# JuliaMolSim/DFTK.jl

Measured on NVIDIA H100. Metric: hpsi_band_applies_per_s, higher is better.
Workload: dtype f64

## Files before the change

### dftk.jl_b200/csrc/fft.cu

```cuda
#include "structs.cuh"

namespace dftk {

#define FFT_THREADS 256
extern __shared__ __align__(16) unsigned char dyn_smem[];

__global__ void __launch_bounds__(FFT_THREADS)
k_sphere_to_x(SphereTables T, FftPlan px, const cplx* twx, const cplx* psi, int64_t ldpsi, cplx* W1,
              int L, int Lp) {
  stage_sphere_to_x(T, px, twx, psi, ldpsi, W1, L, Lp, (cplx*)dyn_smem,
                    Dim3i{(int)blockIdx.x, (int)blockIdx.y, 0});
}
__global__ void __launch_bounds__(FFT_THREADS)
k_y_backward(SphereTables T, FftPlan py, const cplx* twy, const cplx* W1, cplx* W2, int L, int Lp) {
  stage_y_backward(T, py, twy, W1, W2, L, Lp, (cplx*)dyn_smem,
                   Dim3i{(int)blockIdx.x, (int)blockIdx.y, (int)blockIdx.z});
}
__global__ void __launch_bounds__(FFT_THREADS)
k_z_apply_potential(SphereTables T, FftPlan pz, const cplx* twz, cplx* W2, const double* V, int L,
                    int Lp) {
  stage_z_apply_potential(T, pz, twz, W2, V, L, Lp, (cplx*)dyn_smem,
                          Dim3i{(int)blockIdx.x, (int)blockIdx.y, (int)blockIdx.z});
}
__global__ void __launch_bounds__(FFT_THREADS)
// ... 153 lines not shown
  dftk_b200_ctx* ctx = g->ctx;
  ensure_scratch(kb, nb);
  if ((g->rx && kb->T.ranges_ok)) {
    int L = reg_L(g->rx), Lp = L + 1;
    const cplx* tw = (const cplx*)g->twx.p;
    cplx* W1 = kb->W1.p;
    void* args[] = {&kb->T, &tw, &psi, &ldpsi, &W1, &L, &Lp};
    launch_ptr(ctx, g->rx->sphere_to_x, dim3(cdiv(kb->T.n_cols, L), nb), L * g->rx->T, reg_smem(g->rx) + 5 * L * sizeof(int), args);
  } else {
    int L = g->Lx, Lp = L | 1;
    LAUNCH(ctx, k_sphere_to_x, dim3(cdiv(kb->T.n_cols, L), nb), FFT_THREADS, smem_for(g->nx, L), kb->T,
           g->px, (const cplx*)g->twx.p, psi, ldpsi, kb->W1.p, L, Lp);
  }
  if ((g->ry && kb->T.ranges_ok)) {
    int L = reg_L(g->ry), Lp = L + 1;
    const cplx* tw = (const cplx*)g->twy.p;
    const cplx* W1 = kb->W1.p;
    cplx* W2 = kb->W2.p;
    void* args[] = {&kb->T, &tw, &W1, &W2, &L, &Lp};
    launch_ptr(ctx, g->ry->y_backward, dim3(cdiv(g->nx, L), kb->T.n_zc, nb), L * g->ry->T, reg_smem(g->ry), args);
  } else {
    int L = g->Ly, Lp = L | 1;
    LAUNCH(ctx, k_y_backward, dim3(cdiv(g->nx, L), kb->T.n_zc, nb), FFT_THREADS, smem_for(g->ny, L),
           kb->T, g->py, (const cplx*)g->twy.p, (const cplx*)kb->W1.p, kb->W2.p, L, Lp);
  }
}

void kb_planes_to_sphere(dftk_b200_kblock* kb, cplx* out, int64_t ldout, int nb, double scale,
                         const double* kin, const cplx* psi, int64_t ldpsi, int accumulate) {
  dftk_b200_grid* g = kb->grid;
  dftk_b200_ctx* ctx = g->ctx;
  if ((g->ry && kb->T.ranges_ok)) {
    int L = reg_L(g->ry), Lp = L + 1;
    const cplx* tw = (const cplx*)g->twy.p;
    const cplx* W2 = kb->W2.p;
    cplx* W1 = kb->W1.p;
    void* args[] = {&kb->T, &tw, &W2, &W1, &L, &Lp};
    launch_ptr(ctx, g->ry->y_forward, dim3(cdiv(g->nx, L), kb->T.n_zc, nb), L * g->ry->T, reg_smem(g->ry), args);
  } else {
    int L = g->Ly, Lp = L | 1;
    LAUNCH(ctx, k_y_forward, dim3(cdiv(g->nx, L), kb->T.n_zc, nb), FFT_THREADS, smem_for(g->ny, L),
           kb->T, g->py, (const cplx*)g->twy.p, (const cplx*)kb->W2.p, kb->W1.p, L, Lp);
  }
  if ((g->rx && kb->T.ranges_ok)) {
    int L = reg_L(g->rx), Lp = L + 1;
    const cplx* tw = (const cplx*)g->twx.p;
    const cplx* W1 = kb->W1.p;
    void* args[] = {&kb->T, &tw, &W1, &out, &ldout, &scale, &kin, &psi, &ldpsi, &accumulate, &L, &Lp};
    launch_ptr(ctx, g->rx->x_to_sphere, dim3(cdiv(kb->T.n_cols, L), nb), L * g->rx->T, reg_smem(g->rx) + 5 * L * sizeof(int), args);
  } else {
    int L = g->Lx, Lp = L | 1;
    LAUNCH(ctx, k_x_to_sphere, dim3(cdiv(kb->T.n_cols, L), nb), FFT_THREADS, smem_for(g->nx, L), kb->T,
           g->px, (const cplx*)g->twx.p, (const cplx*)kb->W1.p, out, ldout, scale, kin, psi, ldpsi,
           accumulate, L, Lp);
  }
}

void kb_apply_local_kinetic(dftk_b200_kblock* kb, const cplx* psi, cplx* hpsi, int64_t n_bands,
                            bool with_local, bool with_kin, bool accumulate) {
  dftk_b200_grid* g = kb->grid;
  dftk_b200_ctx* ctx = g->ctx;
  if (n_bands == 0) return;
  if (!with_local) {
    scale_kin_add(ctx, psi, hpsi, with_kin ? kb->kin.p : nullptr, kb->n_pw, n_bands, accumulate);
    return;
  }
  REQUIRE(kb->has_V, "apply_h: local potential not set (dftk_b200_kblock_set_potential)");
  const bool fused = kb_yz_fused(kb);
  const int chunk = band_chunk_for(kb, n_bands, !fused);
  for (int64_t b0 = 0; b0 < n_bands; b0 += chunk) {
    int nb = (int)std::min<int64_t>(chunk, n_bands - b0);
    const cplx* p = psi + b0 * kb->n_pw;
    if (fused) {
      kb->W1.ensure((size_t)nb * kb->Th.n_cols * g->nx);
      int L = reg_L(g->rx), Lp = L + 1;
      const size_t sm_x = reg_smem(g->rx) + 5 * L * sizeof(int);
      const cplx* twx = (const cplx*)g->twx.p;
      const cplx* twy = (const cplx*)g->twy.p;
      cplx* W1 = kb->W1.p;
      int64_t ld = kb->n_pw;
      void* a1[] = {&kb->T, &twx, &p, &ld, &W1, &L, &Lp};
      launch_ptr(ctx, g->rx->sphere_to_xt, dim3(cdiv(kb->T.n_cols, L), nb), L * g->rx->T, sm_x, a1);
      const double* Vt = kb->Vtp();
      void* a2[] = {&kb->T, &twy, &W1, &Vt};
      launch_ptr(ctx, g->ry->yz_apply, dim3(nb, g->nx), kYzLines * g->ry->T, yz_smem(g->ny, kb->T.n_zc), a2);
      cplx* out = hpsi + b0 * kb->n_pw;
      double scale = 1.0;
      const double* kin = with_kin ? kb->kin.p : nullptr;
      int acc = accumulate ? 1 : 0;
      void* a3[] = {&kb->T, &twx, &W1, &out, &ld, &scale, &kin, &p, &ld, &acc, &L, &Lp};
      launch_ptr(ctx, g->rx->xt_to_sphere, dim3(cdiv(kb->T.n_cols, L), nb), L * g->rx->T, sm_x, a3);
      continue;
    }
    kb_sphere_to_planes(kb, p, kb->n_pw, nb);
    if ((g->rz && kb->T.ranges_ok)) {
      int L = reg_L(g->rz), Lp = L + 1;
      const cplx* tw = (const cplx*)g->twz.p;
      cplx* W2 = kb->W2.p;
      const double* V = kb->Vp();
      void* args[] = {&kb->T, &tw, &W2, &V, &L, &Lp};
      const size_t sm_pipe = reg_smem(g->rz) / 2 + 2 * (size_t)kb->T.n_zc * L * sizeof(cplx);
      const int64_t n_tiles = (int64_t)cdiv(g->nx, L) * g->ny * nb;
      if (ctx->z_pipeline && sm_pipe <= 100 * 1024 && n_tiles >= 2 * (int64_t)ctx->sm_count) {
        int per_sm = (int)std::min<size_t>(4, (size_t)(220 * 1024) / sm_pipe);
        unsigned grid = (unsigned)std::min<int64_t>(n_tiles, (int64_t)per_sm * ctx->sm_count);
        void* pargs[] = {&kb->T, &tw, &W2, &V, &nb};
        launch_ptr(ctx, g->rz->z_apply_pipe, dim3(grid), L * g->rz->T, sm_pipe, pargs);
      } else {
        launch_ptr(ctx, g->rz->z_apply, dim3(cdiv(g->nx, L), g->ny, nb), L * g->rz->T, reg_smem(g->rz) / 2, args);
      }
    } else {
      int L = g->Lz, Lp = L | 1;
      LAUNCH(ctx, k_z_apply_potential, dim3(cdiv(g->nx, L), g->ny, nb), FFT_THREADS, smem_for(g->nz, L),
             kb->T, g->pz, (const cplx*)g->twz.p, kb->W2.p, (const double*)kb->Vp(), L, Lp);
    }
    kb_planes_to_sphere(kb, hpsi + b0 * kb->n_pw, kb->n_pw, nb, 1.0, with_kin ? kb->kin.p : nullptr, p,
                        kb->n_pw, accumulate ? 1 : 0);
  }
}

bool kb_apply_local_kinetic_multi(int n, dftk_b200_kblock* const* kbs, const cplx* const* psi, cplx* const* hpsi,
                                  const int* n_bands, const void* (*upload)(void* self, const void* host, size_t bytes), void* self) {
  if (n <= 0) return true;
  dftk_b200_grid* g = kbs[0]->grid;
  dftk_b200_ctx* ctx = g->ctx;
  if (!(g->rx && g->ry && g->rz)) return false;
  int total = 0, max_cols = 0, max_zc = 0;
  for (int i = 0; i < n; ++i) {
    dftk_b200_kblock* kb = kbs[i];
    if (kb->grid != g || !kb->T.ranges_ok || !kb->has_V || !kb->has_kin || n_bands[i] <= 0) return false;
    if (band_chunk_for(kb, n_bands[i]) < n_bands[i]) return false;
    total += n_bands[i];
    max_cols = std::max(max_cols, kb->T.n_cols);
    max_zc = std::max(max_zc, kb->T.n_zc);
  }
  if (total > 65535) return false;
  std::vector<FftMultiItem> items(n);
  std::vector<int2> bandmap(total);
  int b = 0;
  for (int i = 0; i < n; ++i) {
    dftk_b200_kblock* kb = kbs[i];
    ensure_scratch(kb, n_bands[i]);
    FftMultiItem& it = items[i];
    it.T = kb->T;
    it.psi = psi[i];
    it.ldpsi = kb->n_pw;
    it.W1 = kb->W1.p;
    it.W2 = kb->W2.p;
    it.V = kb->Vp();
    it.wts = nullptr;
    it.nb = n_bands[i];
    it.out = hpsi[i];
    it.ldout = kb->n_pw;
    it.kin = kb->kin.p;
    for (int l = 0; l < n_bands[i]; ++l) bandmap[b++] = make_int2(i, l);
  }
  const FftMultiItem* d_items = (const FftMultiItem*)upload(self, items.data(), items.size() * sizeof(FftMultiItem));
  const int2* d_map = (const int2*)upload(self, bandmap.data(), bandmap.size() * sizeof(int2));
  {
    int L = reg_L(g->rx), Lp = L + 1;
    const cplx* tw = (const cplx*)g->twx.p;
    void* args[] = {&d_items, &d_map, &tw, &L, &Lp};
    launch_ptr(ctx, g->rx->m_sphere_to_x, dim3(cdiv(max_cols, L), total), L * g->rx->T, reg_smem(g->rx) + 5 * L * sizeof(int), args);
  }
  {
    int L = reg_L(g->ry), Lp = L + 1;
    const cplx* tw = (const cplx*)g->twy.p;
    void* args[] = {&d_items, &d_map, &tw, &L, &Lp};
// ... 184 lines not shown
```

### dftk.jl_b200/csrc/fft_core.cuh

```cuda
#pragma once
#include <cuda_runtime.h>
#include <stdint.h>

#if defined(__CUDA_ARCH__)
#define TLOOP(t, n) for (int t = threadIdx.x; t < (n); t += blockDim.x)
#define TSYNC() __syncthreads()
#else
#define TLOOP(t, n) for (int t = 0; t < (n); ++t)
#define TSYNC() ((void)0)
#endif
#if defined(__CUDA_ARCH__)
#define TLOOPC(t, n, nthr)                                                        \
  _Pragma("unroll") for (int i__ = 0; i__ < ((n) + (nthr)-1) / (nthr); ++i__)    \
      for (int t = (int)threadIdx.x + i__ * (nthr), once__ = 1; once__ && t < (n); once__ = 0)
#define TLOOPU(t, n) _Pragma("unroll 4") for (int t = threadIdx.x; t < (n); t += blockDim.x)
#else
#define TLOOPC(t, n, nthr) for (int t = 0; t < (n); ++t)
#define TLOOPU(t, n) for (int t = 0; t < (n); ++t)
#endif
#define HD __host__ __device__ __forceinline__

namespace dftk {

typedef double2 cplx;

HD cplx cmul(cplx a, cplx b) { return make_double2(a.x * b.x - a.y * b.y, a.x * b.y + a.y * b.x); }
HD cplx cadd(cplx a, cplx b) { return make_double2(a.x + b.x, a.y + b.y); }
HD cplx csub(cplx a, cplx b) { return make_double2(a.x - b.x, a.y - b.y); }
HD cplx cscale(cplx a, double s) { return make_double2(a.x * s, a.y * s); }
HD cplx cmuli(cplx a, double s) { return make_double2(-s * a.y, s * a.x); }

#define DFTK_MAX_PASSES 12
struct FftPlan {
  int n;
  int npass;
  int radix[DFTK_MAX_PASSES];
};

HD cplx twiddle(const cplx* __restrict__ tw, int m, int sign) {
  cplx w = tw[m];
  if (sign > 0) w.y = -w.y;
  return w;
}

template <int R>
HD void butterfly(cplx* v, int sign) {
  const double s = (double)sign;
  if (R == 2) {
    cplx a = v[0], b = v[1];
    v[0] = cadd(a, b);
    v[1] = csub(a, b);
  } else if (R == 4) {
    cplx t0 = cadd(v[0], v[2]), t1 = csub(v[0], v[2]);
    cplx t2 = cadd(v[1], v[3]), t3 = cmuli(csub(v[1], v[3]), s);
    v[0] = cadd(t0, t2);
    v[2] = csub(t0, t2);
    v[1] = cadd(t1, t3);
    v[3] = csub(t1, t3);
  } else if (R == 3) {
    const double h = 0.86602540378443864676;
    cplx t1 = cadd(v[1], v[2]);
    cplx m = make_double2(v[0].x - 0.5 * t1.x, v[0].y - 0.5 * t1.y);
    cplx d = cmuli(cscale(csub(v[1], v[2]), h), s);
    v[0] = cadd(v[0], t1);
    v[1] = cadd(m, d);
    v[2] = csub(m, d);
  } else if (R == 5) {
    const double c1 = 0.30901699437494742410, c2 = -0.80901699437494742410;
    const double s1 = 0.95105651629515357212, s2 = 0.58778525229247312917;
    cplx t1 = cadd(v[1], v[4]), t2 = cadd(v[2], v[3]);
    cplx t3 = csub(v[1], v[4]), t4 = csub(v[2], v[3]);
    cplx m1 = make_double2(v[0].x + c1 * t1.x + c2 * t2.x, v[0].y + c1 * t1.y + c2 * t2.y);
    cplx m2 = make_double2(v[0].x + c2 * t1.x + c1 * t2.x, v[0].y + c2 * t1.y + c1 * t2.y);
    cplx n1 = cmuli(make_double2(s1 * t3.x + s2 * t4.x, s1 * t3.y + s2 * t4.y), s);
    cplx n2 = cmuli(make_double2(s2 * t3.x - s1 * t4.x, s2 * t3.y - s1 * t4.y), s);
    v[0] = cadd(v[0], cadd(t1, t2));
    v[1] = cadd(m1, n1);
    v[4] = csub(m1, n1);
    v[2] = cadd(m2, n2);
    v[3] = csub(m2, n2);
  }
}

template <int R>
HD void stockham_pass(const cplx* __restrict__ in, cplx* __restrict__ out, int n, int Ns, int L,
                      int Lp, const cplx* __restrict__ tw, int sign) {
  const int nb = n / R;
  const int tstep = n / (Ns * R);
  TLOOP(t, nb * L) {
    int line = t % L, j = t / L;
    int k = j % Ns;
    cplx v[R];
#pragma unroll
    for (int r = 0; r < R; ++r) {
      cplx x = in[(j + r * nb) * Lp + line];
      v[r] = (r == 0 || k == 0) ? x : cmul(x, twiddle(tw, r * k * tstep, sign));
    }
    butterfly<R>(v, sign);
    int j0 = (j / Ns) * Ns * R + k;
#pragma unroll
    for (int r = 0; r < R; ++r) out[(j0 + r * Ns) * Lp + line] = v[r];
// ... 325 lines not shown
```

### dftk.jl_b200/csrc/fft_reg.cu

```cuda
#include "structs.cuh"
#include "fft_reg.cuh"

#ifndef REG_GROUP
#define REG_GROUP 0
#endif
#ifndef REG_NGROUPS
#define REG_NGROUPS 1
#endif

namespace dftk {

extern __shared__ __align__(16) unsigned char dyn_smem_reg[];
#define REG_MAXT(A, B) (32 * ((A) > (B) ? (A) : (B)))

template <int A, int B, int XM>
__global__ void __launch_bounds__(REG_MAXT(A, B))
kr_sphere_to_x(SphereTablesX T, const cplx* tw, const cplx* psi, int64_t ldpsi, cplx* W1, int L, int Lp) {
  reg_sphere_to_x<A, B, XM>(T, tw, psi, ldpsi, W1, L, Lp, (cplx*)dyn_smem_reg, Dim3i{(int)blockIdx.x, (int)blockIdx.y, 0});
}
template <int A, int B>
__global__ void __launch_bounds__(REG_MAXT(A, B))
kr_y_backward(SphereTablesX T, const cplx* tw, const cplx* W1, cplx* W2, int L, int Lp) {
  reg_y_backward<A, B>(T, tw, W1, W2, L, Lp, (cplx*)dyn_smem_reg, Dim3i{(int)blockIdx.x, (int)blockIdx.y, (int)blockIdx.z});
}
template <int A, int B>
__global__ void __launch_bounds__(REG_MAXT(A, B))
kr_z_apply(SphereTablesX T, const cplx* tw, cplx* W2, const double* V, int L, int Lp) {
  reg_z_apply_potential<A, B>(T, tw, W2, V, L, Lp, (cplx*)dyn_smem_reg, Dim3i{(int)blockIdx.x, (int)blockIdx.y, (int)blockIdx.z});
}
template <int A, int B>
__global__ void __launch_bounds__(REG_MAXT(A, B))
kr_z_apply_pipe(SphereTablesX T, const cplx* tw, cplx* W2, const double* V, int n_bands) {
  reg_z_apply_potential_pipe<A, B>(T, tw, W2, V, (cplx*)dyn_smem_reg, n_bands);
}
template <int A, int B>
__global__ void __launch_bounds__(REG_MAXT(A, B))
kr_z_to_cube(SphereTablesX T, const cplx* tw, const cplx* W2, cplx* cube, double scale, int L, int Lp) {
  reg_z_to_cube<A, B>(T, tw, W2, cube, scale, L, Lp, (cplx*)dyn_smem_reg, Dim3i{(int)blockIdx.x, (int)blockIdx.y, (int)blockIdx.z});
}
template <int A, int B>
__global__ void __launch_bounds__(REG_MAXT(A, B))
kr_z_from_cube(SphereTablesX T, const cplx* tw, const cplx* cube, cplx* W2, int L, int Lp) {
  reg_z_from_cube<A, B>(T, tw, cube, W2, L, Lp, (cplx*)dyn_smem_reg, Dim3i{(int)blockIdx.x, (int)blockIdx.y, (int)blockIdx.z});
}
template <int A, int B>
__global__ void __launch_bounds__(REG_MAXT(A, B))
kr_z_density(SphereTablesX T, const cplx* tw, const cplx* W2, const double* wts, int nb, double* rho, int L, int Lp) {
  reg_z_density<A, B>(T, tw, W2, wts, nb, rho, L, Lp, (cplx*)dyn_smem_reg, Dim3i{(int)blockIdx.x, (int)blockIdx.y, 0});
}
template <int A, int B>
__global__ void __launch_bounds__(REG_MAXT(A, B))
kr_y_forward(SphereTablesX T, const cplx* tw, const cplx* W2, cplx* W1, int L, int Lp) {
  reg_y_forward<A, B>(T, tw, W2, W1, L, Lp, (cplx*)dyn_smem_reg, Dim3i{(int)blockIdx.x, (int)blockIdx.y, (int)blockIdx.z});
}
template <int A, int B, int XM>
__global__ void __launch_bounds__(REG_MAXT(A, B))
kr_x_to_sphere(SphereTablesX T, const cplx* tw, const cplx* W1, cplx* out, int64_t ldout, double scale,
               const double* kin, const cplx* psi, int64_t ldpsi, int accumulate, int L, int Lp) {
  reg_x_to_sphere<A, B, XM>(T, tw, W1, out, ldout, scale, kin, psi, ldpsi, accumulate, L, Lp, (cplx*)dyn_smem_reg,
                        Dim3i{(int)blockIdx.x, (int)blockIdx.y, 0});
}
template <int A, int B>
__global__ void __launch_bounds__(RegYZ<A, B>::LL * RegYZ<A, B>::T, 1)
kr_yz_apply(SphereTablesX T, const cplx* tw, cplx* W1t, const double* Vt) {
  reg_yz_apply<A, B>(T, tw, W1t, Vt, (cplx*)dyn_smem_reg, Dim3i{(int)blockIdx.y, 0, (int)blockIdx.x});
}

template <int A, int B>
__global__ void __launch_bounds__(REG_MAXT(A, B))
kr_sphere_to_x_multi(const FftMultiItem* __restrict__ items, const int2* __restrict__ bandmap, const cplx* tw, int L, int Lp) {
  const int2 bm = bandmap[blockIdx.y];
  const FftMultiItem& it = items[bm.x];
  if ((int)blockIdx.x * L >= it.T.n_cols) return;
  reg_sphere_to_x<A, B>(it.T, tw, it.psi, it.ldpsi, it.W1, L, Lp, (cplx*)dyn_smem_reg, Dim3i{(int)blockIdx.x, bm.y, 0});
}
template <int A, int B>
__global__ void __launch_bounds__(REG_MAXT(A, B))
kr_y_backward_multi(const FftMultiItem* __restrict__ items, const int2* __restrict__ bandmap, const cplx* tw, int L, int Lp) {
  const int2 bm = bandmap[blockIdx.z];
  const FftMultiItem& it = items[bm.x];
  if ((int)blockIdx.y >= it.T.n_zc) return;
  reg_y_backward<A, B>(it.T, tw, it.W1, it.W2, L, Lp, (cplx*)dyn_smem_reg, Dim3i{(int)blockIdx.x, (int)blockIdx.y, bm.y});
}
template <int A, int B>
__global__ void __launch_bounds__(REG_MAXT(A, B))
kr_z_apply_multi(const FftMultiItem* __restrict__ items, const int2* __restrict__ bandmap, const cplx* tw, int L, int Lp) {
  const int2 bm = bandmap[blockIdx.z];
  const FftMultiItem& it = items[bm.x];
  reg_z_apply_potential<A, B>(it.T, tw, it.W2, it.V, L, Lp, (cplx*)dyn_smem_reg, Dim3i{(int)blockIdx.x, (int)blockIdx.y, bm.y});
}
template <int A, int B>
__global__ void __launch_bounds__(REG_MAXT(A, B))
kr_y_forward_multi(const FftMultiItem* __restrict__ items, const int2* __restrict__ bandmap, const cplx* tw, int L, int Lp) {
  const int2 bm = bandmap[blockIdx.z];
  const FftMultiItem& it = items[bm.x];
  if ((int)blockIdx.y >= it.T.n_zc) return;
  reg_y_forward<A, B>(it.T, tw, it.W2, it.W1, L, Lp, (cplx*)dyn_smem_reg, Dim3i{(int)blockIdx.x, (int)blockIdx.y, bm.y});
}
template <int A, int B>
__global__ void __launch_bounds__(REG_MAXT(A, B))
kr_x_to_sphere_multi(const FftMultiItem* __restrict__ items, const int2* __restrict__ bandmap, const cplx* tw, int L, int Lp) {
  const int2 bm = bandmap[blockIdx.y];
  const FftMultiItem& it = items[bm.x];
  if ((int)blockIdx.x * L >= it.T.n_cols) return;
  reg_x_to_sphere<A, B>(it.T, tw, it.W1, it.out, it.ldout, 1.0, it.kin, it.psi, it.ldpsi, 0, L, Lp, (cplx*)dyn_smem_reg,
                        Dim3i{(int)blockIdx.x, bm.y, 0});
}

template <int A, int B>
__global__ void __launch_bounds__(REG_MAXT(A, B))
kr_z_density_multi(const FftMultiItem* __restrict__ items, int n_items, int spin, const cplx* tw, double* rho, int L, int Lp) {
  for (int i = 0; i < n_items; ++i) {
    const FftMultiItem& it = items[i];
    if ((int)(intptr_t)it.kin != spin) continue;
    reg_z_density<A, B>(it.T, tw, it.W2, it.wts, it.nb, rho, L, Lp, (cplx*)dyn_smem_reg, Dim3i{(int)blockIdx.x, (int)blockIdx.y, 0});
    __syncthreads();
  }
}

template <int A, int B>
static RegKernels make_entry() {
  RegKernels k;
  k.A = A;
  k.B = B;
  k.T = RegPair<A, B>::T;
  k.sphere_to_x = (const void*)kr_sphere_to_x<A, B, 0>;
  k.sphere_to_xt = (const void*)kr_sphere_to_x<A, B, 1>;
  k.y_backward = (const void*)kr_y_backward<A, B>;
  k.z_apply = (const void*)kr_z_apply<A, B>;
  k.z_apply_pipe = (const void*)kr_z_apply_pipe<A, B>;
  k.z_to_cube = (const void*)kr_z_to_cube<A, B>;
  k.z_from_cube = (const void*)kr_z_from_cube<A, B>;
  k.z_density = (const void*)kr_z_density<A, B>;
  k.y_forward = (const void*)kr_y_forward<A, B>;
  k.x_to_sphere = (const void*)kr_x_to_sphere<A, B, 0>;
  k.xt_to_sphere = (const void*)kr_x_to_sphere<A, B, 1>;
  k.yz_apply = (const void*)kr_yz_apply<A, B>;
  k.m_sphere_to_x = (const void*)kr_sphere_to_x_multi<A, B>;
  k.m_y_backward = (const void*)kr_y_backward_multi<A, B>;
  k.m_z_apply = (const void*)kr_z_apply_multi<A, B>;
  k.m_y_forward = (const void*)kr_y_forward_multi<A, B>;
  k.m_x_to_sphere = (const void*)kr_x_to_sphere_multi<A, B>;
  k.m_z_density = (const void*)kr_z_density_multi<A, B>;
  return k;
}

#define REG_CONCAT2(a, b) a##b
#define REG_CONCAT(a, b) REG_CONCAT2(a, b)
void REG_CONCAT(reg_register_group_, REG_GROUP)(std::vector<RegKernels>& out) {
  int idx = 0;
#define DFTK_X(a, b)                                          \
  if ((idx++ % REG_NGROUPS) == REG_GROUP) out.push_back(make_entry<a, b>());
  DFTK_REG_PAIRS(DFTK_X)
#undef DFTK_X
}

}
```

### dftk.jl_b200/csrc/fft_reg.cuh

```cuda
#pragma once
#include "fft_core.cuh"
#include "fft_reg_fwd.cuh"
#include "fft_radix_gen.cuh"

namespace dftk {

template <int A, int B>
struct RegPair {
  static constexpr int n = A * B;
  static constexpr int T = (A > B ? A : B);
  static constexpr int L = (T >= 12 ? 8 : (T >= 5 ? 16 : 32));
  static constexpr int Lp = L + 1;
};

template <int A, int B, int S>
HD void pass1_store(const cplx* x, int q, int line, cplx* __restrict__ Sbuf, int Lp,
                    const cplx* __restrict__ tw) {
  cplx Y[A];
  dft_r<A, S>(x, Y);
#pragma unroll
  for (int c = 0; c < A; ++c) {
    cplx v = Y[c];
    if (c != 0 && q != 0) v = cmul(v, twiddle(tw, q * c, S));
    Sbuf[(c * B + q) * Lp + line] = v;
// ... 282 lines not shown
  TLOOP(t, n * L) {
    const int line = t % L, iz = t / L, x = x0 + line;
    if (x < nx) rho[((size_t)iz * ny + y) * nx + x] += acc[t];
  }
}

template <int A, int B>
HD void reg_y_backward(const SphereTablesX& T, const cplx* __restrict__ tw, const cplx* __restrict__ W1,
                       cplx* __restrict__ W2, int L_rt, int Lp_rt, cplx* sm, Dim3i bid) {
  constexpr int n = A * B, TT = RegPair<A, B>::T, L = RegPair<A, B>::L, Lp = RegPair<A, B>::Lp;
  (void)L_rt;
  (void)Lp_rt;
  const int nx = T.nx;
  cplx* bufA = sm;
  const int x0 = bid.x * L, izc = bid.y;
  const cplx* in = W1 + (size_t)bid.z * T.n_cols * nx;
  cplx* out = W2 + ((size_t)bid.z * T.n_zc + izc) * n * nx;
  const PlaneCols pc = plane_cols(T, izc);
  TLOOP(t, L * TT) {
    const int line = t % L, p = t / L, x = x0 + line;
    if (p < B) {
      cplx v[A];
#pragma unroll
      for (int r = 0; r < A; ++r) {
        int c = pc.col(p + B * r);
        v[r] = ld_pred(in + (unsigned)((c < 0 ? 0 : c) * nx + x), c >= 0 && x < nx);
      }
      pass1_store<A, B, +1>(v, p, line, bufA, Lp, tw);
    }
  }
  TSYNC();
  TLOOP(t, L * TT) {
    const int line = t % L, p = t / L, x = x0 + line;
    if (p < A) {
      cplx X[B];
      pass2_load<A, B, +1>(X, p, line, bufA, Lp);
#pragma unroll
      for (int d = 0; d < B; ++d)
        st_pred(out + (unsigned)((p + A * d) * nx + x), X[d], x < nx);
    }
  }
}

template <int A, int B>
HD void reg_y_forward(const SphereTablesX& T, const cplx* __restrict__ tw, const cplx* __restrict__ W2,
                      cplx* __restrict__ W1, int L_rt, int Lp_rt, cplx* sm, Dim3i bid) {
  constexpr int n = A * B, TT = RegPair<A, B>::T, L = RegPair<A, B>::L, Lp = RegPair<A, B>::Lp;
  (void)L_rt;
  (void)Lp_rt;
  const int nx = T.nx;
  cplx* bufA = sm;
  const int x0 = bid.x * L, izc = bid.y;
  const cplx* in = W2 + ((size_t)bid.z * T.n_zc + izc) * n * nx;
  cplx* out = W1 + (size_t)bid.z * T.n_cols * nx;
  const PlaneCols pc = plane_cols(T, izc);
  TLOOP(t, L * TT) {
    const int line = t % L, p = t / L, x = x0 + line;
    if (p < B) {
      cplx v[A];
#pragma unroll
      for (int r = 0; r < A; ++r)
        v[r] = ld_pred(in + (unsigned)((p + B * r) * nx + x), x < nx);
      pass1_store<A, B, -1>(v, p, line, bufA, Lp, tw);
    }
  }
  TSYNC();
  TLOOP(t, L * TT) {
    const int line = t % L, p = t / L, x = x0 + line;
    if (p < A) {
      cplx X[B];
      pass2_load<A, B, -1>(X, p, line, bufA, Lp);
#pragma unroll
      for (int d = 0; d < B; ++d) {
        int c = pc.col(p + A * d);
        st_pred(out + (unsigned)((c < 0 ? 0 : c) * nx + x), X[d], c >= 0 && x < nx);
      }
    }
  }
}

template <int A, int B>
struct RegYZ {
  static constexpr int n = A * B, T = RegPair<A, B>::T, LL = 25, Sy = n | 1;
  static size_t smem(int n_zc) { return ((size_t)n_zc + (DFTK_Z_ALIAS ? 1 : 2) * LL) * Sy * sizeof(cplx); }
};

template <int A, int B>
HD void reg_yz_apply(const SphereTablesX& T, const cplx* __restrict__ tw, cplx* __restrict__ W1t,
                     const double* __restrict__ Vt, cplx* sm, Dim3i bid) {
  constexpr int n = A * B, TT = RegYZ<A, B>::T, LL = RegYZ<A, B>::LL, Sy = RegYZ<A, B>::Sy;
  const int n_zc = T.n_zc, x = bid.x;
  cplx* S = sm;
  cplx* E = sm + (size_t)n_zc * Sy;
  cplx* E2 = DFTK_Z_ALIAS ? E : E + (size_t)LL * Sy;
  cplx* row = W1t + ((size_t)bid.z * T.nx + x) * T.n_cols;
  const double* vx = Vt + (size_t)x * n * n;
  const uint64_t pol_keep = l2_policy_evict_last();
  for (int zc0 = 0; zc0 < n_zc; zc0 += LL) {
    TLOOP(t, LL * TT) {
      const int line = t % LL, p = t / LL, zc = zc0 + line;
      if (p < B && zc < n_zc) {
        const PlaneCols pc = plane_cols(T, zc);
        cplx v[A];
#pragma unroll
        for (int r = 0; r < A; ++r) {
          int c = pc.col(p + B * r);
          v[r] = ld_pred(row + (c < 0 ? 0 : c), c >= 0);
        }
        pass1_store<A, B, +1>(v, p, 0, E + line * Sy, 1, tw);
      }
    }
    TSYNC();
    TLOOP(t, LL * TT) {
      const int line = t % LL, p = t / LL, zc = zc0 + line;
      if (p < A && zc < n_zc) {
        cplx X[B];
        pass2_load<A, B, +1>(X, p, 0, E + line * Sy, 1);
#pragma unroll
        for (int d = 0; d < B; ++d) S[zc * Sy + p + A * d] = X[d];
      }
    }
    TSYNC();
  }
  for (int y0 = 0; y0 < n; y0 += LL) {
    TLOOP(t, LL * TT) {
      const int line = t % LL, p = t / LL, y = y0 + line;
      if (p < B && y < n) {
        cplx v[A];
#pragma unroll
        for (int r = 0; r < A; ++r) {
          int zc = zc_index(T, p + B * r);
          v[r] = zc >= 0 ? S[zc * Sy + y] : make_double2(0.0, 0.0);
        }
        pass1_store<A, B, +1>(v, p, 0, E + line * Sy, 1, tw);
      }
    }
    TSYNC();
    TLOOP(t, LL * TT) {
      const int line = t % LL, p = t / LL, y = y0 + line;
      cplx Y[B];
      if (p < A && y < n) {
        cplx X[B];
        pass2_load<A, B, +1>(X, p, 0, E + line * Sy, 1);
#pragma unroll
        for (int d = 0; d < B; ++d) X[d] = cscale(X[d], ld_pred_hint(vx + y * n + p + A * d, true, pol_keep));
        pass1_compute<B, A, -1>(X, p, tw, Y);
      }
#if DFTK_Z_ALIAS
      __syncthreads();
#endif
      if (p < A && y < n) {
#pragma unroll
        for (int c = 0; c < B; ++c) E2[line * Sy + c * A + p] = Y[c];
      }
    }
    TSYNC();
    TLOOP(t, LL * TT) {
      const int line = t % LL, p = t / LL, y = y0 + line;
      if (p < B && y < n) {
        cplx X[A];
        pass2_load<B, A, -1>(X, p, 0, E2 + line * Sy, 1);
#pragma unroll
        for (int f = 0; f < A; ++f) {
          int zc = zc_index(T, p + B * f);
          if (zc >= 0) S[zc * Sy + y] = X[f];
        }
      }
    }
    TSYNC();
  }
  for (int zc0 = 0; zc0 < n_zc; zc0 += LL) {
    TLOOP(t, LL * TT) {
      const int line = t % LL, p = t / LL, zc = zc0 + line;
      if (p < B && zc < n_zc) {
        cplx v[A];
#pragma unroll
        for (int r = 0; r < A; ++r) v[r] = S[zc * Sy + p + B * r];
        pass1_store<A, B, -1>(v, p, 0, E + line * Sy, 1, tw);
      }
    }
    TSYNC();
    TLOOP(t, LL * TT) {
      const int line = t % LL, p = t / LL, zc = zc0 + line;
      if (p < A && zc < n_zc) {
        const PlaneCols pc = plane_cols(T, zc);
        cplx X[B];
        pass2_load<A, B, -1>(X, p, 0, E + line * Sy, 1);
#pragma unroll
        for (int d = 0; d < B; ++d) {
          int c = pc.col(p + A * d);
          st_pred(row + (c < 0 ? 0 : c), X[d], c >= 0);
        }
      }
    }
    TSYNC();
  }
}

HD void load_col_desc(const SphereTablesX& T, int c0, int L, int* cd) {
  TLOOP(t, L) {
    int c = c0 + t;
    bool ok = c < T.n_cols;
    cd[5 * t + 0] = ok ? T.col_start[c] : 0;
    cd[5 * t + 1] = ok ? T.cx_n0[c] : 0;
    cd[5 * t + 2] = ok ? T.cx_s0[c] : 0;
    cd[5 * t + 3] = ok ? T.cx_n1[c] : 0;
    cd[5 * t + 4] = ok ? T.cx_s1[c] : 0;
  }
}

template <int n, int L, int XM>
HD void w1_index(int t, int& line, int& x) {
  line = XM ? t % L : t / n;
  x = XM ? t / L : t % n;
}
template <int n, int XM>
HD size_t w1_offset(int c, int x, int n_cols) {
  return XM ? (size_t)x * n_cols + c : (size_t)c * n + x;
}

template <int A, int B, int XM = 0>
HD void reg_sphere_to_x(const SphereTablesX& T, const cplx* __restrict__ tw, const cplx* __restrict__ psi,
                        int64_t ldpsi, cplx* __restrict__ W1, int L_rt, int Lp_rt, cplx* sm, Dim3i bid) {
  constexpr int n = A * B, TT = RegPair<A, B>::T, L = RegPair<A, B>::L, Lp = RegPair<A, B>::Lp;
  (void)L_rt;
  (void)Lp_rt;
  cplx* bufA = sm;
  cplx* bufB = sm + (size_t)n * Lp;
  int* cd = (int*)(sm + 2 * (size_t)n * Lp);
  const int c0 = bid.x * L;
  const int64_t band = bid.y;
  load_col_desc(T, c0, L, cd);
  TLOOPC(t, n * Lp, L * TT) bufA[t] = make_double2(0.0, 0.0);
  TSYNC();
  const cplx* pb = psi + band * ldpsi;
  TLOOPC(t, L * n, L * TT) {
    const int line = t / n, i = t % n;
    const int n0 = cd[5 * line + 1], n1 = cd[5 * line + 3];
    if (i < n0 + n1) {
      const int ix = i < n0 ? cd[5 * line + 2] + i : cd[5 * line + 4] + (i - n0);
      bufA[ix * Lp + line] = pb[cd[5 * line] + i];
    }
  }
  TSYNC();
  TLOOP(t, L * TT) {
    const int line = t % L, p = t / L;
    if (p < B) {
      cplx v[A];
#pragma unroll
      for (int r = 0; r < A; ++r) v[r] = bufA[(p + B * r) * Lp + line];
      pass1_store<A, B, +1>(v, p, line, bufB, Lp, tw);
    }
  }
  TSYNC();
  TLOOP(t, L * TT) {
    const int line = t % L, p = t / L;
    if (p < A) {
      cplx X[B];
      pass2_load<A, B, +1>(X, p, line, bufB, Lp);
#pragma unroll
      for (int d = 0; d < B; ++d) bufA[(p + A * d) * Lp + line] = X[d];
    }
  }
  TSYNC();
  cplx* out = W1 + (size_t)band * T.n_cols * n;
  TLOOPC(t, L * n, L * TT) {
    int line, x;
    w1_index<n, L, XM>(t, line, x);
    const int c = c0 + line;
    if (c < T.n_cols) out[w1_offset<n, XM>(c, x, T.n_cols)] = bufA[x * Lp + line];
  }
}

template <int A, int B, int XM = 0>
HD void reg_x_to_sphere(const SphereTablesX& T, const cplx* __restrict__ tw, const cplx* __restrict__ W1,
                        cplx* __restrict__ out, int64_t ldout, double scale, const double* __restrict__ kin,
                        const cplx* __restrict__ psi, int64_t ldpsi, int accumulate, int L_rt, int Lp_rt, cplx* sm,
                        Dim3i bid) {
// ... 64 lines not shown
```

### dftk.jl_b200/csrc/structs.cuh

```cuda
#pragma once
#include "common.cuh"
#include "fft_reg_fwd.cuh"
#include "fft_plan.h"

namespace dftk {
struct SphereTablesX;
struct RegKernels {
  int A, B, T;
  const void *sphere_to_x, *y_backward, *z_apply, *z_to_cube, *z_from_cube, *z_density, *y_forward, *x_to_sphere;
  const void* z_apply_pipe;
  const void* yz_apply;
  const void *sphere_to_xt, *xt_to_sphere;
  const void *m_sphere_to_x, *m_y_backward, *m_z_apply, *m_y_forward, *m_x_to_sphere, *m_z_density;
};
struct FftMultiItem {
  SphereTablesX T;
  const cplx* psi;
  long long ldpsi;
  cplx *W1, *W2;
  const double* V;
  cplx* out;
  long long ldout;
  const double* kin;
  const double* wts;
  int nb;
};
const RegKernels* reg_kernels_for(int n);
void reg_set_attributes(int smem_optin);
}

namespace dftk {
struct I8Operand {
  const signed char* planes = nullptr;
  const int* exps = nullptr;
  int64_t cols = 0, k = 0, ldk = 0;
  int n_mod = 0;
};
}

struct dftk_b200_grid {
  dftk_b200_ctx* ctx;
  int nx, ny, nz;
  int64_t N;
  double omega;
  double ifft_norm, fft_norm;
  dftk::FftPlan px, py, pz;
  dftk::DevBuf<double> twx, twy, twz;
  int Lx, Ly, Lz;
  const dftk::RegKernels *rx = nullptr, *ry = nullptr, *rz = nullptr;
  dftk::DevBuf<double> Vs[2];
  dftk::DevBuf<double> Vts[2];
  bool has_Vs[2] = {false, false};
};

struct dftk_b200_kblock {
  dftk_b200_grid* grid;
  int64_t n_pw, n_proj;
  int spin;
  double kweight;
  dftk::SphereTablesHost Th;
  dftk::SphereTablesX T;
  dftk::DevBuf<int> d_col_start, d_col_cnt, d_slot_ix, d_slot_src, d_zlist, d_colmap, d_zc_of, d_pl_s0, d_pl_n0, d_pl_s1, d_pl_n1, d_pl_col0, d_cx_s0, d_cx_n0, d_cx_s1,
      d_cx_n1;
  dftk::DevBuf<double> kin;
  bool has_kin = false;
  dftk::DevBuf<dftk::cplx> P;
  std::vector<double> D_host;
  dftk::DevBuf<dftk::cplx> Dc;
  int64_t n_orb = 0;
  dftk::DevBuf<dftk::cplx> Dh;
  std::vector<int64_t> map_h;
  int64_t n_nl() const { return n_proj + n_orb; }
  const dftk::cplx* Dnl() const { return n_orb ? Dh.p : Dc.p; }
  dftk::DevBuf<signed char> i8_pool[8];
  dftk::DevBuf<int> i8_epool[8];
  dftk::I8Operand i8_Pop;
  dftk::DevBuf<signed char> i8_psi_planes;
  dftk::DevBuf<int> i8_psi_exps;
  dftk::DevBuf<signed char> i8_planes;
  dftk::DevBuf<int> i8_exps;
  dftk::DevBuf<dftk::cplx> PD;
  int64_t n_half = 0;
  dftk::DevBuf<int> fold_i, fold_p;
  dftk::DevBuf<double> R;
  dftk::DevBuf<dftk::cplx> fold_ws;
  dftk::DevBuf<double> V;
  bool has_V = false;
  int grid_V = -1;
  const double* Vp() const { return grid_V >= 0 ? grid->Vs[grid_V].p : V.p; }
  dftk::DevBuf<double> Vt;
  const double* Vtp() const { return grid_V >= 0 ? grid->Vts[grid_V].p : Vt.p; }
// ... 94 lines not shown
```

Before: 11090.

## Split fused yz kernel into independent warp groups with named barriers and persistent grid

The fused y/z FFT-and-potential kernel now splits each CTA into up to three warp groups. Each group processes its own slice of z-columns or y-lines with a small exchange buffer and synchronises through named barriers (bar.sync with a per-group id) instead of block-wide __syncthreads, so groups advance without waiting on each other. The launch becomes a persistent grid sized from the occupancy query, and each CTA loops over (x, band) items. This is meant to cut block-wide barrier stalls and launch imbalance, at the cost of an occupancy query on every call and possible load imbalance when work does not split evenly across groups.

```diff
diff --git a/dftk.jl_b200/csrc/fft.cu b/dftk.jl_b200/csrc/fft.cu
--- a/dftk.jl_b200/csrc/fft.cu
+++ b/dftk.jl_b200/csrc/fft.cu
@@ -259,8 +259,12 @@
       void* a1[] = {&kb->T, &twx, &p, &ld, &W1, &L, &Lp};
       launch_ptr(ctx, g->rx->sphere_to_xt, dim3(cdiv(kb->T.n_cols, L), nb), L * g->rx->T, sm_x, a1);
       const double* Vt = kb->Vtp();
-      void* a2[] = {&kb->T, &twy, &W1, &Vt};
-      launch_ptr(ctx, g->ry->yz_apply, dim3(nb, g->nx), kYzLines * g->ry->T, yz_smem(g->ny, kb->T.n_zc), a2);
+      void* a2[] = {&kb->T, &twy, &W1, &Vt, &nb};
+      const size_t sm_yz = yz_smem(g->ny, kb->T.n_zc);
+      int per_sm = 1;
+      CUDA_CHECK(cudaOccupancyMaxActiveBlocksPerMultiprocessor(&per_sm, g->ry->yz_apply, g->ry->yz_threads, sm_yz));
+      const unsigned yz_ctas = (unsigned)std::min<int64_t>((int64_t)nb * g->nx, (int64_t)std::max(per_sm, 1) * ctx->sm_count);
+      launch_ptr(ctx, g->ry->yz_apply, dim3(yz_ctas), g->ry->yz_threads, sm_yz, a2);
       cplx* out = hpsi + b0 * kb->n_pw;
       double scale = 1.0;
       const double* kin = with_kin ? kb->kin.p : nullptr;
diff --git a/dftk.jl_b200/csrc/fft_core.cuh b/dftk.jl_b200/csrc/fft_core.cuh
--- a/dftk.jl_b200/csrc/fft_core.cuh
+++ b/dftk.jl_b200/csrc/fft_core.cuh
@@ -17,6 +17,20 @@
 #else
 #define TLOOPC(t, n, nthr) for (int t = 0; t < (n); ++t)
 #define TLOOPU(t, n) for (int t = 0; t < (n); ++t)
+#endif
+__device__ __forceinline__ int tid_volatile() {
+  int t;
+  asm volatile("mov.u32 %0, %%tid.x;" : "=r"(t));
+  return t;
+}
+#if defined(__CUDA_ARCH__)
+#define GLOOP(g, G, GT) for (int g = (int)threadIdx.x / (GT), gonce__ = 1; gonce__; gonce__ = 0)
+#define GTLOOP(t, GT) for (int t = tid_volatile() % (GT), tonce__ = 1; tonce__; tonce__ = 0)
+#define GSYNC(g, GT) asm volatile("bar.sync %0, %1;" ::"r"(1 + (g)), "r"(GT) : "memory")
+#else
+#define GLOOP(g, G, GT) for (int g = 0; g < (G); ++g)
+#define GTLOOP(t, GT) for (int t = 0; t < (GT); ++t)
+#define GSYNC(g, GT) ((void)(g))
 #endif
 #define HD __host__ __device__ __forceinline__
 
diff --git a/dftk.jl_b200/csrc/fft_reg.cu b/dftk.jl_b200/csrc/fft_reg.cu
--- a/dftk.jl_b200/csrc/fft_reg.cu
+++ b/dftk.jl_b200/csrc/fft_reg.cu
@@ -61,9 +61,11 @@
                         Dim3i{(int)blockIdx.x, (int)blockIdx.y, 0});
 }
 template <int A, int B>
-__global__ void __launch_bounds__(RegYZ<A, B>::LL * RegYZ<A, B>::T, 1)
-kr_yz_apply(SphereTablesX T, const cplx* tw, cplx* W1t, const double* Vt) {
-  reg_yz_apply<A, B>(T, tw, W1t, Vt, (cplx*)dyn_smem_reg, Dim3i{(int)blockIdx.y, 0, (int)blockIdx.x});
+__global__ void __launch_bounds__(RegYZ<A, B>::NT, 1)
+kr_yz_apply(SphereTablesX T, const cplx* tw, cplx* W1t, const double* Vt, int nb) {
+  const int n_items = nb * T.nx;
+  for (int i = blockIdx.x; i < n_items; i += gridDim.x)
+    reg_yz_apply<A, B>(T, tw, W1t, Vt, (cplx*)dyn_smem_reg, Dim3i{i / nb, 0, i % nb});
 }
 
 template <int A, int B>
@@ -124,6 +126,7 @@
   k.A = A;
   k.B = B;
   k.T = RegPair<A, B>::T;
+  k.yz_threads = RegYZ<A, B>::NT;
   k.sphere_to_x = (const void*)kr_sphere_to_x<A, B, 0>;
   k.sphere_to_xt = (const void*)kr_sphere_to_x<A, B, 1>;
   k.y_backward = (const void*)kr_y_backward<A, B>;
diff --git a/dftk.jl_b200/csrc/fft_reg.cuh b/dftk.jl_b200/csrc/fft_reg.cuh
--- a/dftk.jl_b200/csrc/fft_reg.cuh
+++ b/dftk.jl_b200/csrc/fft_reg.cuh
@@ -388,118 +388,135 @@
 template <int A, int B>
 struct RegYZ {
   static constexpr int n = A * B, T = RegPair<A, B>::T, LL = 25, Sy = n | 1;
+  static constexpr int GL = 8, GW = (GL * T + 31) / 32;
+  static constexpr int G = (12 / GW < 3 ? 12 / GW : 3), GT = 32 * GW, NT = G * GT;
+  static_assert(G >= 1 && G * GL <= LL, "the groups' exchange lines must fit the buffer");
   static size_t smem(int n_zc) { return ((size_t)n_zc + (DFTK_Z_ALIAS ? 1 : 2) * LL) * Sy * sizeof(cplx); }
 };
 
 template <int A, int B>
 HD void reg_yz_apply(const SphereTablesX& T, const cplx* __restrict__ tw, cplx* __restrict__ W1t,
                      const double* __restrict__ Vt, cplx* sm, Dim3i bid) {
-  constexpr int n = A * B, TT = RegYZ<A, B>::T, LL = RegYZ<A, B>::LL, Sy = RegYZ<A, B>::Sy;
+  constexpr int n = A * B, LL = RegYZ<A, B>::LL, Sy = RegYZ<A, B>::Sy;
+  constexpr int GL = RegYZ<A, B>::GL, G = RegYZ<A, B>::G, GT = RegYZ<A, B>::GT;
   const int n_zc = T.n_zc, x = bid.x;
   cplx* S = sm;
-  cplx* E = sm + (size_t)n_zc * Sy;
-  cplx* E2 = DFTK_Z_ALIAS ? E : E + (size_t)LL * Sy;
   cplx* row = W1t + ((size_t)bid.z * T.nx + x) * T.n_cols;
   const double* vx = Vt + (size_t)x * n * n;
   const uint64_t pol_keep = l2_policy_evict_last();
-  for (int zc0 = 0; zc0 < n_zc; zc0 += LL) {
-    TLOOP(t, LL * TT) {
-      const int line = t % LL, p = t / LL, zc = zc0 + line;
-      if (p < B && zc < n_zc) {
-        const PlaneCols pc = plane_cols(T, zc);
-        cplx v[A];
-#pragma unroll
-        for (int r = 0; r < A; ++r) {
-          int c = pc.col(p + B * r);
-          v[r] = ld_pred(row + (c < 0 ? 0 : c), c >= 0);
-        }
-        pass1_store<A, B, +1>(v, p, 0, E + line * Sy, 1, tw);
-      }
-    }
-    TSYNC();
-    TLOOP(t, LL * TT) {
-      const int line = t % LL, p = t / LL, zc = zc0 + line;
-      if (p < A && zc < n_zc) {
-        cplx X[B];
-        pass2_load<A, B, +1>(X, p, 0, E + line * Sy, 1);
-#pragma unroll
-        for (int d = 0; d < B; ++d) S[zc * Sy + p + A * d] = X[d];
-      }
-    }
-    TSYNC();
-  }
-  for (int y0 = 0; y0 < n; y0 += LL) {
-    TLOOP(t, LL * TT) {
-      const int line = t % LL, p = t / LL, y = y0 + line;
-      if (p < B && y < n) {
-        cplx v[A];
-#pragma unroll
-        for (int r = 0; r < A; ++r) {
-          int zc = zc_index(T, p + B * r);
-          v[r] = zc >= 0 ? S[zc * Sy + y] : make_double2(0.0, 0.0);
-        }
-        pass1_store<A, B, +1>(v, p, 0, E + line * Sy, 1, tw);
-      }
-    }
-    TSYNC();
-    TLOOP(t, LL * TT) {
-      const int line = t % LL, p = t / LL, y = y0 + line;
-      cplx Y[B];
-      if (p < A && y < n) {
-        cplx X[B];
-        pass2_load<A, B, +1>(X, p, 0, E + line * Sy, 1);
-#pragma unroll
-        for (int d = 0; d < B; ++d) X[d] = cscale(X[d], ld_pred_hint(vx + y * n + p + A * d, true, pol_keep));
-        pass1_compute<B, A, -1>(X, p, tw, Y);
-      }
+  GLOOP(g, G, GT) {
+    cplx* E = sm + ((size_t)n_zc + g * GL) * Sy;
+    const int zc1 = (g + 1) * n_zc / G;
+    for (int zc0 = g * n_zc / G; zc0 < zc1; zc0 += GL) {
+      GTLOOP(t, GT) {
+        const int line = t % GL, p = t / GL, zc = zc0 + line;
+        if (p < B && zc < zc1) {
+          const PlaneCols pc = plane_cols(T, zc);
+          cplx v[A];
+#pragma unroll
+          for (int r = 0; r < A; ++r) {
+            int c = pc.col(p + B * r);
+            v[r] = ld_pred(row + (c < 0 ? 0 : c), c >= 0);
+          }
+          pass1_store<A, B, +1>(v, p, 0, E + line * Sy, 1, tw);
+        }
+      }
+      GSYNC(g, GT);
+      GTLOOP(t, GT) {
+        const int line = t % GL, p = t / GL, zc = zc0 + line;
+        if (p < A && zc < zc1) {
+          cplx X[B];
+          pass2_load<A, B, +1>(X, p, 0, E + line * Sy, 1);
+#pragma unroll
+          for (int d = 0; d < B; ++d) S[zc * Sy + p + A * d] = X[d];
+        }
+      }
+      GSYNC(g, GT);
+    }
+  }
+  TSYNC();
+  GLOOP(g, G, GT) {
+    cplx* E = sm + ((size_t)n_zc + g * GL) * Sy;
+    cplx* E2 = DFTK_Z_ALIAS ? E : E + (size_t)LL * Sy;
+    const int y1 = (g + 1) * n / G;
+    for (int y0 = g * n / G; y0 < y1; y0 += GL) {
+      GTLOOP(t, GT) {
+        const int line = t % GL, p = t / GL, y = y0 + line;
+        if (p < B && y < y1) {
+          cplx v[A];
+#pragma unroll
+          for (int r = 0; r < A; ++r) {
+            int zc = zc_index(T, p + B * r);
+            v[r] = zc >= 0 ? S[zc * Sy + y] : make_double2(0.0, 0.0);
+          }
+          pass1_store<A, B, +1>(v, p, 0, E + line * Sy, 1, tw);
+        }
+      }
+      GSYNC(g, GT);
+      GTLOOP(t, GT) {
+        const int line = t % GL, p = t / GL, y = y0 + line;
+        cplx Y[B];
+        if (p < A && y < y1) {
+          cplx X[B];
+          pass2_load<A, B, +1>(X, p, 0, E + line * Sy, 1);
+#pragma unroll
+          for (int d = 0; d < B; ++d) X[d] = cscale(X[d], ld_pred_hint(vx + y * n + p + A * d, true, pol_keep));
+          pass1_compute<B, A, -1>(X, p, tw, Y);
+        }
 #if DFTK_Z_ALIAS
-      __syncthreads();
+        GSYNC(g, GT);
 #endif
-      if (p < A && y < n) {
-#pragma unroll
-        for (int c = 0; c < B; ++c) E2[line * Sy + c * A + p] = Y[c];
-      }
-    }
-    TSYNC();
-    TLOOP(t, LL * TT) {
-      const int line = t % LL, p = t / LL, y = y0 + line;
-      if (p < B && y < n) {
-        cplx X[A];
-        pass2_load<B, A, -1>(X, p, 0, E2 + line * Sy, 1);
-#pragma unroll
-        for (int f = 0; f < A; ++f) {
-          int zc = zc_index(T, p + B * f);
-          if (zc >= 0) S[zc * Sy + y] = X[f];
-        }
-      }
-    }
-    TSYNC();
-  }
-  for (int zc0 = 0; zc0 < n_zc; zc0 += LL) {
-    TLOOP(t, LL * TT) {
-      const int line = t % LL, p = t / LL, zc = zc0 + line;
-      if (p < B && zc < n_zc) {
-        cplx v[A];
-#pragma unroll
-        for (int r = 0; r < A; ++r) v[r] = S[zc * Sy + p + B * r];
-        pass1_store<A, B, -1>(v, p, 0, E + line * Sy, 1, tw);
-      }
-    }
-    TSYNC();
-    TLOOP(t, LL * TT) {
-      const int line = t % LL, p = t / LL, zc = zc0 + line;
-      if (p < A && zc < n_zc) {
-        const PlaneCols pc = plane_cols(T, zc);
-        cplx X[B];
-        pass2_load<A, B, -1>(X, p, 0, E + line * Sy, 1);
-#pragma unroll
-        for (int d = 0; d < B; ++d) {
-          int c = pc.col(p + A * d);
-          st_pred(row + (c < 0 ? 0 : c), X[d], c >= 0);
-        }
-      }
-    }
-    TSYNC();
+        if (p < A && y < y1) {
+#pragma unroll
+          for (int c = 0; c < B; ++c) E2[line * Sy + c * A + p] = Y[c];
+        }
+      }
+      GSYNC(g, GT);
+      GTLOOP(t, GT) {
+        const int line = t % GL, p = t / GL, y = y0 + line;
+        if (p < B && y < y1) {
+          cplx X[A];
+          pass2_load<B, A, -1>(X, p, 0, E2 + line * Sy, 1);
+#pragma unroll
+          for (int f = 0; f < A; ++f) {
+            int zc = zc_index(T, p + B * f);
+            if (zc >= 0) S[zc * Sy + y] = X[f];
+          }
+        }
+      }
+      GSYNC(g, GT);
+    }
+  }
+  TSYNC();
+  GLOOP(g, G, GT) {
+    cplx* E = sm + ((size_t)n_zc + g * GL) * Sy;
+    const int zc1 = (g + 1) * n_zc / G;
+    for (int zc0 = g * n_zc / G; zc0 < zc1; zc0 += GL) {
+      GTLOOP(t, GT) {
+        const int line = t % GL, p = t / GL, zc = zc0 + line;
+        if (p < B && zc < zc1) {
+          cplx v[A];
+#pragma unroll
+          for (int r = 0; r < A; ++r) v[r] = S[zc * Sy + p + B * r];
+          pass1_store<A, B, -1>(v, p, 0, E + line * Sy, 1, tw);
+        }
+      }
+      GSYNC(g, GT);
+      GTLOOP(t, GT) {
+        const int line = t % GL, p = t / GL, zc = zc0 + line;
+        if (p < A && zc < zc1) {
+          const PlaneCols pc = plane_cols(T, zc);
+          cplx X[B];
+          pass2_load<A, B, -1>(X, p, 0, E + line * Sy, 1);
+#pragma unroll
+          for (int d = 0; d < B; ++d) {
+            int c = pc.col(p + A * d);
+            st_pred(row + (c < 0 ? 0 : c), X[d], c >= 0);
+          }
+        }
+      }
+      GSYNC(g, GT);
+    }
   }
 }
 
diff --git a/dftk.jl_b200/csrc/structs.cuh b/dftk.jl_b200/csrc/structs.cuh
--- a/dftk.jl_b200/csrc/structs.cuh
+++ b/dftk.jl_b200/csrc/structs.cuh
@@ -7,6 +7,7 @@
 struct SphereTablesX;
 struct RegKernels {
   int A, B, T;
+  int yz_threads;
   const void *sphere_to_x, *y_backward, *z_apply, *z_to_cube, *z_from_cube, *z_density, *y_forward, *x_to_sphere;
   const void* z_apply_pipe;
   const void* yz_apply;
```

Measured after the change: 11940 (median of 6 runs). +7.7%, better.
